# Tycro-Games/Raytracer-VoxPopuli

Hardware: AMD Instinct MI355X
Metric: Mray/s (primary+shadow) at 1920×1080, 1024³ world; 1/2/4/8-GPU (higher is better)
Workload: dtype f32

## Files before the change

raytracer-voxpopuli_amd/csrc/vpx_skip.hpp:

```cpp
#pragma once

#include <stdint.h>

#ifndef __HIP_DEVICE_COMPILE__
#include <cstring>
#endif

#if defined(__HIPCC__)
#define VPX_HD __host__ __device__ __forceinline__
#else
#define VPX_HD inline
#endif

namespace vpx {
namespace skip {

VPX_HD uint32_t fbits(float f) {
#if defined(__HIP_DEVICE_COMPILE__)
    return __float_as_uint(f);
#else
    uint32_t u;
    std::memcpy(&u, &f, 4);
    return u;
#endif
// ... 397 lines not shown
    return step1_commit(w, n, ax, ay, az);
}

VPX_HD int skip_box(Walk& w, const uint32_t lo[3], const uint32_t hi[3], float bound, uint32_t& cells) {
    const float h[3] = {w.tx, w.ty, w.tz};
    const float d[3] = {w.dx, w.dy, w.dz};
    const int32_t s[3] = {w.sx, w.sy, w.sz};
    const uint32_t c[3] = {w.X, w.Y, w.Z};
    uint32_t e[3];
    float approx[3];
    for (int k = 0; k < 3; ++k) {
        if (!(h[k] > 0.0f) || !(d[k] > 0.0f)) return 2;
        e[k] = s[k] > 0 ? hi[k] - c[k] + 1u : c[k] - lo[k] + 1u;
        approx[k] = e[k] > 1u ? h[k] + (float)(e[k] - 1u) * d[k] : h[k];
    }
    float V[3], Vp[3];
    bool exact[3] = {false, false, false};
    int a = (approx[2] <= approx[0] && approx[2] <= approx[1]) ? 2 : (approx[1] <= approx[0] ? 1 : 0);
    const float amin = approx[a];
    bool close = false;
    for (int k = 0; k < 3; ++k)
        if (k != a && !(approx[k] > amin * 1.0003f)) close = true;
    if (close) {
        for (int k = 0; k < 3; ++k) {
            count_below2(h[k], d[k], 3.4e38f, true, e[k] - 1u, V[k], Vp[k]);
            exact[k] = true;
        }
        a = (V[2] <= V[0] && V[2] <= V[1]) ? 2 : (V[1] <= V[0] ? 1 : 0);
    } else {
        count_below2(h[a], d[a], 3.4e38f, true, e[a] - 1u, V[a], Vp[a]);
        exact[a] = true;
    }
    const float vs = V[a];
    uint32_t nk[3];
    float head[3], prev[3];
    for (int k = 0; k < 3; ++k) {
        if (k == a) {
            nk[k] = e[k] - 1u;
            head[k] = V[k];
            prev[k] = Vp[k];
        } else {
            nk[k] = count_below2(h[k], d[k], vs, k < a, e[k] - 1u, head[k], prev[k]);
        }
    }
    if (vs < bound) {
        float tl = w.t;
        bool moved = false;
        for (int k = 0; k < 3; ++k) {
            if (nk[k] == 0) continue;
            tl = moved ? (tl < prev[k] ? prev[k] : tl) : prev[k];
            moved = true;
        }
        if (moved) w.t = tl;
        w.tx = head[0], w.ty = head[1], w.tz = head[2];
        w.X += nk[0] * (uint32_t)w.sx;
        w.Y += nk[1] * (uint32_t)w.sy;
        w.Z += nk[2] * (uint32_t)w.sz;
        cells += nk[0] + nk[1] + nk[2];
        return 0;
    }
    uint32_t v = 1u;
    for (int k = 0; k < 3; ++k) v += count_below(h[k], d[k], bound, true, nk[k]);
    cells += v;
    return 1;
}


VPX_HD uint32_t mul24(uint32_t a, uint32_t b) {
#if defined(__HIP_DEVICE_COMPILE__)
    return __umul24(a, b);
#else
    return a * b;
#endif
}

VPX_HD uint32_t mad24(uint32_t a, uint32_t b, uint32_t c) {
#if defined(__HIP_DEVICE_COMPILE__)
    uint32_t r;
    asm("v_mad_u32_u24 %0, %1, %2, %3" : "=v"(r) : "v"(a), "v"(b), "v"(c));
    return r;
#else
    return a * b + c;
#endif
}


VPX_HD float rcp_approx(float x) {
#if defined(__HIP_DEVICE_COMPILE__)
    return __builtin_amdgcn_rcpf(x);
#else
    return 1.0f / x;
#endif
}

VPX_HD bool seg_params_nb(float a, float d, uint32_t& b, uint32_t& c, uint32_t& e) {
    const uint32_t ab = fbits(a), db = fbits(d);
    const uint32_t ea = ab >> 23, ed = db >> 23;
    const uint32_t sh = ea - ed;
    const uint32_t sh1 = sh > 1u ? sh : 1u, shc = sh1 < 24u ? sh1 : 24u;
    const uint32_t md = (db & 0x7fffffu) | 0x800000u;
    const uint32_t rem = md & ((1u << shc) - 1u), half = 1u << (shc - 1u);
    const uint32_t c0 = md >> shc;
    const uint32_t b0 = (ab & 0x7fffffu) | 0x800000u;
    const bool tie = rem == half;
    c = tie ? c0 + (c0 & 1u) : c0 + (rem > half ? 1u : 0u);
    b = tie ? b0 + ((b0 + c0) & 1u) - (c0 & 1u) : b0;
    e = ea;
    return (ea - 1u < 254u) & (ed - 1u < 254u) & (sh - 1u < 24u) & (c != 0u);
}

VPX_HD uint32_t ceil_div_cap_r(uint32_t p, uint32_t c, float rc) {
    const float q = (float)p * rc;
    uint32_t j = (uint32_t)(q < 1024.5f ? q : 1024.5f) + 1u;
    j -= mul24(j - 1u, c) >= p ? 1u : 0u;
    j += mul24(j, c) < p ? 1u : 0u;
    return j < 1025u ? j : 1025u;
}
VPX_HD uint32_t ceil_div_cap(uint32_t p, uint32_t c) { return ceil_div_cap_r(p, c, rcp_approx((float)c)); }

VPX_HD uint32_t floor_div_cap_r(uint32_t r, uint32_t c, float rc) {
    const float q = (float)r * rc;
    uint32_t m = (uint32_t)(q < 1024.5f ? q : 1024.5f);
    m -= ((m != 0u) & (mul24(m, c) > r)) ? 1u : 0u;
    m += mul24(m + 1u, c) <= r ? 1u : 0u;
    return m < 1024u ? m : 1024u;
}
VPX_HD uint32_t floor_div_cap(uint32_t r, uint32_t c) { return floor_div_cap_r(r, c, rcp_approx((float)c)); }

VPX_HD uint32_t seg_first_cap(uint32_t b, uint32_t c, uint32_t e, float T, bool strict) {
    const uint32_t tb = fbits(T), te = tb >> 23;
    const uint32_t need = ((tb & 0x7fffffu) | 0x800000u) + (strict ? 0u : 1u);
    const uint32_t q = ceil_div_cap(need - b, c);
    const uint32_t f = need <= b ? 0u : q;
    return te == e ? f : (te < e ? 0u : 1025u);
}

struct Axis {
    uint32_t b1, c1, e1, m1, b2, c2, e2, l;
};

VPX_HD bool seg_immature(float h, float d) {
    const uint32_t ea = fbits(h) >> 23, ed = fbits(d) >> 23;
    return (ea - 1u < 254u) & (ed - 1u < 254u) & (ed >= ea);
}
template <bool PRE = false>
VPX_HD bool axis_seg1(float h, float d, Axis& a, uint32_t& fit1) {
    const bool ok1 = seg_params_nb(h, d, a.b1, a.c1, a.e1);
    if (PRE) a.c1 = ok1 ? a.c1 : 1u;
    const uint32_t room = a.b1 <= 0xffffffu ? 0xffffffu - a.b1 : 0u;
    fit1 = floor_div_cap(room, a.c1 ? a.c1 : 1u);
    if (PRE) fit1 = ok1 ? fit1 : 0u;
    a.b2 = 0u, a.c2 = 1u, a.e2 = 0u;
    return PRE ? ok1 | seg_immature(h, d) : ok1;
}
template <bool PRE = false>
VPX_HD uint32_t axis_seg2(float h, float d, Axis& a, uint32_t fit1) {
    const uint32_t amc = (a.e1 << 23) | (mad24(fit1, a.c1, a.b1) & 0x7fffffu);
    const uint32_t am = fit1 ? amc : fbits(h);
    const float A = bitsf(am) + d;
    uint32_t b2;
    const bool ok2 = seg_params_nb(A, d, b2, a.c2, a.e2);
    const bool exact2 = b2 == ((fbits(A) & 0x7fffffu) | 0x800000u);
    a.b2 = b2;
    if (PRE) a.c2 = ok2 ? a.c2 : 1u;
    const uint32_t room2 = b2 <= 0xffffffu ? 0xffffffu - b2 : 0u;
    const uint32_t fit2 = floor_div_cap(room2, a.c2 ? a.c2 : 1u);
    if (PRE) return exact2 ? fit1 + 1u + (ok2 ? fit2 : 0u) : fit1;
    return (ok2 & exact2) ? fit1 + 1u + fit2 : fit1;
}
VPX_HD void axis_clip(Axis& a, uint32_t l, bool ok1, uint32_t reach, uint32_t fit1) {
    const uint32_t lim = ok1 ? reach : 0u;
    a.l = l < lim ? l : lim;
    a.m1 = a.l < fit1 ? a.l : fit1;
}
VPX_HD float axis_head2(const Axis& a) { return bitsf((a.e2 << 23) | (a.b2 & 0x7fffffu)); }
VPX_HD bool axis_outrun(const Axis& a, uint32_t want) { return (want > a.l) & (a.l > a.m1); }
VPX_HD uint32_t axis_rebase(float& h, float d, Axis& a, uint32_t want, bool on) {
    const uint32_t fit1 = a.m1, fit2 = a.l - fit1 - 1u;
    const float A = bitsf((a.e2 << 23) | (mad24(fit2, a.c2, a.b2) & 0x7fffffu)) + d;
    uint32_t b3, c3, e3;
    const bool ok3 = seg_params_nb(A, d, b3, c3, e3);
    const bool exact3 = b3 == ((fbits(A) & 0x7fffffu) | 0x800000u);
    const uint32_t room3 = b3 <= 0xffffffu ? 0xffffffu - b3 : 0u;
    const uint32_t fit3 = floor_div_cap(room3, c3 ? c3 : 1u);
    const bool go = on & axis_outrun(a, want) & ok3 & exact3;
    const uint32_t off = fit1 + 1u, l = want - off, lim = fit2 + 1u + fit3;
    h = go ? axis_head2(a) : h;
    a.b1 = go ? a.b2 : a.b1, a.c1 = go ? a.c2 : a.c1, a.e1 = go ? a.e2 : a.e1;
    a.b2 = go ? b3 : a.b2, a.c2 = go ? c3 : a.c2, a.e2 = go ? e3 : a.e2;
    a.l = go ? (l < lim ? l : lim) : a.l;
    a.m1 = go ? (a.l < fit2 ? a.l : fit2) : a.m1;
    return go ? off : 0u;
}
VPX_HD bool any_lane(bool b) {
#if defined(__HIP_DEVICE_COMPILE__)
    return __ballot(b) != 0ull;
#else
    return b;
#endif
}

template <bool PRE = false>
VPX_HD void axis_setup(float h, float d, uint32_t l, Axis& a) {
    const bool ok1 = seg_params_nb(h, d, a.b1, a.c1, a.e1);
    if (PRE) a.c1 = ok1 ? a.c1 : 1u;
    const uint32_t room = a.b1 <= 0xffffffu ? 0xffffffu - a.b1 : 0u;
    const uint32_t fit1q = floor_div_cap(room, a.c1 ? a.c1 : 1u);
    const uint32_t fit1 = PRE && !ok1 ? 0u : fit1q;
    const uint32_t amc = (a.e1 << 23) | (mad24(fit1, a.c1, a.b1) & 0x7fffffu);
    const uint32_t am = fit1 ? amc : fbits(h);
    const float A = bitsf(am) + d;
    uint32_t b2;
    const bool ok2 = seg_params_nb(A, d, b2, a.c2, a.e2);
    const bool exact2 = b2 == ((fbits(A) & 0x7fffffu) | 0x800000u);
    a.b2 = b2;
    if (PRE) a.c2 = ok2 ? a.c2 : 1u;
    const uint32_t room2 = b2 <= 0xffffffu ? 0xffffffu - b2 : 0u;
    const uint32_t fit2 = floor_div_cap(room2, a.c2 ? a.c2 : 1u);
    const uint32_t reach = PRE ? (exact2 ? fit1 + 1u + (ok2 ? fit2 : 0u) : fit1) : ((ok2 & exact2) ? fit1 + 1u + fit2 : fit1);
    const uint32_t lim = (PRE ? ok1 | seg_immature(h, d) : ok1) ? reach : 0u;
    a.l = l < lim ? l : lim;
    a.m1 = a.l < fit1 ? a.l : fit1;
}

VPX_HD float axis_at(const Axis& a, float h, uint32_t i) {
    const bool one = i <= a.m1;
    const uint32_t b1 = mad24(i, a.c1, a.b1), b2 = mad24(i - a.m1 - 1u, a.c2, a.b2);
    const uint32_t v = ((one ? a.e1 : a.e2) << 23) | ((one ? b1 : b2) & 0x7fffffu);
    return bitsf(i ? v : fbits(h));
}

VPX_HD uint32_t axis_count(const Axis& a, float h, float T, bool strict, uint32_t cap) {
    const bool h_below = strict ? h < T : h <= T;
    const bool s2 = (fbits(T) >> 23) > a.e1;
    uint32_t f = seg_first_cap(s2 ? a.b2 : a.b1, s2 ? a.c2 : a.c1, s2 ? a.e2 : a.e1, T, strict);
    f = s2 ? a.m1 + 1u + f : (f < a.m1 + 1u ? f : a.m1 + 1u);
    f = h_below ? (f > 1u ? f : 1u) : 0u;
    return f < cap ? f : cap;
}

template <bool SEG2_BRANCH = true, int MORE = 0, bool PRE = false>
VPX_HD int skip_box_lean(Walk& w, uint32_t lo[3], uint32_t hi[3], float bound, uint32_t& cells) {
    static_assert(MORE == 0 || SEG2_BRANCH, "skip_box_lean: further segments build on the branch form");
    if (!((w.tx > 0.0f) & (w.ty > 0.0f) & (w.tz > 0.0f))) return 2;
    Axis ax, ay, az;
    if (SEG2_BRANCH) {
    const uint32_t wx = w.sx > 0 ? hi[0] - w.X : w.X - lo[0], wy = w.sy > 0 ? hi[1] - w.Y : w.Y - lo[1],
                   wz = w.sz > 0 ? hi[2] - w.Z : w.Z - lo[2];
    uint32_t fx, fy, fz;
    const bool okx = axis_seg1<PRE>(w.tx, w.dx, ax, fx), oky = axis_seg1<PRE>(w.ty, w.dy, ay, fy),
               okz = axis_seg1<PRE>(w.tz, w.dz, az, fz);
    uint32_t rx = fx, ry = fy, rz = fz;
    if (any_lane((okx & (wx > fx)) | (oky & (wy > fy)) | (okz & (wz > fz)))) {
        rx = axis_seg2<PRE>(w.tx, w.dx, ax, fx);
        ry = axis_seg2<PRE>(w.ty, w.dy, ay, fy);
        rz = axis_seg2<PRE>(w.tz, w.dz, az, fz);
    }
    axis_clip(ax, wx, okx, rx, fx);
    axis_clip(ay, wy, oky, ry, fy);
    axis_clip(az, wz, okz, rz, fz);
    } else {
    axis_setup<PRE>(w.tx, w.dx, w.sx > 0 ? hi[0] - w.X : w.X - lo[0], ax);
    axis_setup<PRE>(w.ty, w.dy, w.sy > 0 ? hi[1] - w.Y : w.Y - lo[1], ay);
    axis_setup<PRE>(w.tz, w.dz, w.sz > 0 ? hi[2] - w.Z : w.Z - lo[2], az);
    }
    for (int more = 0; more < MORE; ++more) {
        const uint32_t wx = w.sx > 0 ? hi[0] - w.X : w.X - lo[0], wy = w.sy > 0 ? hi[1] - w.Y : w.Y - lo[1],
                       wz = w.sz > 0 ? hi[2] - w.Z : w.Z - lo[2];
        const bool ux = axis_outrun(ax, wx), uy = axis_outrun(ay, wy), uz = axis_outrun(az, wz);
        if (!any_lane(ux | uy | uz)) break;
        const float Vx = axis_at(ax, w.tx, ax.l), Vy = axis_at(ay, w.ty, ay.l), Vz = axis_at(az, w.tz, az.l);
        const float Vm = Vx < Vy ? Vx : Vy, Vn = Vm < Vz ? Vm : Vz, T2 = Vn < bound ? Vn : bound;
        const uint32_t ox = axis_rebase(w.tx, w.dx, ax, wx, axis_head2(ax) < T2);
        const uint32_t oy = axis_rebase(w.ty, w.dy, ay, wy, axis_head2(ay) < T2);
        const uint32_t oz = axis_rebase(w.tz, w.dz, az, wz, axis_head2(az) < T2);
        w.X += ox * (uint32_t)w.sx;
        w.Y += oy * (uint32_t)w.sy;
        w.Z += oz * (uint32_t)w.sz;
        cells += ox + oy + oz;
    }
    const uint32_t lx = ax.l, ly = ay.l, lz = az.l;
    if (w.sx > 0) hi[0] = w.X + lx; else lo[0] = w.X - lx;
    if (w.sy > 0) hi[1] = w.Y + ly; else lo[1] = w.Y - ly;
    if (w.sz > 0) hi[2] = w.Z + lz; else lo[2] = w.Z - lz;
    const float Vx = axis_at(ax, w.tx, lx), Vy = axis_at(ay, w.ty, ly), Vz = axis_at(az, w.tz, lz);
    const int a = (Vz <= Vx && Vz <= Vy) ? 2 : (Vy <= Vx ? 1 : 0);
    const float vs = a == 2 ? Vz : (a == 1 ? Vy : Vx);
    const bool inside = vs < bound;
    const float T = inside ? vs : bound;
    uint32_t nx = axis_count(ax, w.tx, T, true, lx);
    uint32_t ny = axis_count(ay, w.ty, T, inside ? a == 2 : true, ly);
    uint32_t nz = axis_count(az, w.tz, T, inside ? false : true, lz);
    if (inside) {
        nx = a == 0 ? lx : nx;
        ny = a == 1 ? ly : ny;
        nz = a == 2 ? lz : nz;
        const float px = axis_at(ax, w.tx, nx - 1u), py = axis_at(ay, w.ty, ny - 1u), pz = axis_at(az, w.tz, nz - 1u);
        float tl = nx ? px : w.t;
        tl = ny ? ((nx && !(tl < py)) ? tl : py) : tl;
        tl = nz ? (((nx | ny) && !(tl < pz)) ? tl : pz) : tl;
        w.t = tl;
        w.tx = axis_at(ax, w.tx, nx), w.ty = axis_at(ay, w.ty, ny), w.tz = axis_at(az, w.tz, nz);
        w.X += nx * (uint32_t)w.sx;
        w.Y += ny * (uint32_t)w.sy;
        w.Z += nz * (uint32_t)w.sz;
        cells += nx + ny + nz;
        return 0;
    }
    const uint32_t cx = a == 0 ? lx : axis_count(ax, w.tx, vs, true, lx);
    const uint32_t cy = a == 1 ? ly : axis_count(ay, w.ty, vs, a == 2, ly);
    const uint32_t cz = a == 2 ? lz : axis_count(az, w.tz, vs, false, lz);
    cells += 1u + (nx < cx ? nx : cx) + (ny < cy ? ny : cy) + (nz < cz ? nz : cz);
    return 1;
}

VPX_HD bool gate_immature(float t, float d, uint32_t G) { return (fbits(t) >> 23) < (fbits(d) >> 23) + G; }
VPX_HD bool gate_open(float tx, float ty, float tz, float dx, float dy, float dz, uint32_t G, uint32_t N) {
    const bool xd = (dx <= dy) & (dx <= dz), yd = !xd & (dy <= dz);
    const float lim = (xd ? tx : (yd ? ty : tz)) + (float)N * (xd ? dx : (yd ? dy : dz));
    const bool ix = gate_immature(tx, dx, G), iy = gate_immature(ty, dy, G), iz = gate_immature(tz, dz, G);
    return !((ix & (tx < lim)) | (iy & (ty < lim)) | (iz & (tz < lim)));
}
VPX_HD uint32_t gate_word(uint32_t G, uint32_t f) { return 1u | G << 1 | f << 3; }
VPX_HD bool gate_open(const Walk& w, uint32_t gate) {
    return !(gate & 1u) || gate_open(w.tx, w.ty, w.tz, w.dx, w.dy, w.dz, (gate >> 1) & 3u, 4u << ((gate >> 3) & 3u));
}

constexpr uint32_t kGatePre = 1u << 8;
constexpr uint32_t kGatePacked = 1u << 9;
template <bool PRE>
VPX_HD int skip_box_lean_more(Walk& w, uint32_t lo[3], uint32_t hi[3], float bound, uint32_t& cells, uint32_t more) {
    return more == 0u   ? skip_box_lean<true, 0, PRE>(w, lo, hi, bound, cells)
           : more == 1u ? skip_box_lean<true, 1, PRE>(w, lo, hi, bound, cells)
           : more == 2u ? skip_box_lean<true, 2, PRE>(w, lo, hi, bound, cells)
           : more == 3u ? skip_box_lean<true, 3, PRE>(w, lo, hi, bound, cells)
                        : skip_box_lean<true, 4, PRE>(w, lo, hi, bound, cells);
}
VPX_HD bool walk_skip(const GridView& g, Walk& w, float bound, uint32_t& cells, uint32_t gate = 0u) {
    const bool wide = g.dfw != nullptr, axes = wide || g.dfa != nullptr;
    const uint32_t axis = dom_axis(w), sec = wide ? sec_axis(w) : 3u;
    const uint32_t apar = plane_parent(g, (w.osh >> 3) * 3u + axis);
    const bool packed = wide && (gate & kGatePacked);
    const uint32_t sel = packed ? box_sel(axis, sec) : 0u;
    for (;;) {
        if (!(w.t < bound)) return false;
        const int cls = axes ? classify_axis_o(w, g, apar) : classify(w, g);
        if (cls == 0) {
            ++cells;
            return true;
        }
        if (cls == 2 && gate_open(w, gate)) {
            uint32_t lo[3], hi[3];
            if (packed) df_box_sel(w, g.n, (uint32_t)w.m1, sel, lo, hi);
            else if (axes) df_box_axis(w, g.n, cube_dfp(w), len_dfa(w), axis, lo, hi, sec, wide ? wid_dfw(w, axis, sec) : 0u);
            else df_box(w, g.n, cube_l1(w), lo, hi);
            const int sr = (gate & kGatePre) ? skip_box_lean_more<true>(w, lo, hi, bound, cells, (gate >> 5) & 7u)
                                             : skip_box_lean_more<false>(w, lo, hi, bound, cells, (gate >> 5) & 7u);
            if (sr == 1) return false;
        }
        ++cells;
        if (!step1(w, g.n)) return false;
    }
}

template <class Occ, class Get>
VPX_HD uint8_t df_value(uint32_t x, uint32_t y, uint32_t z, uint32_t o, uint32_t nb1, Occ occ, Get get) {
    const int32_t s[3] = {(o & 1u) ? -1 : 1, (o & 2u) ? -1 : 1, (o & 4u) ? -1 : 1};
    uint32_t mn = 255;
    for (uint32_t j = 1; j < 8; ++j) {
        const uint32_t a = x + ((j & 1u) ? (uint32_t)s[0] : 0u), b = y + ((j & 2u) ? (uint32_t)s[1] : 0u),
                       c = z + ((j & 4u) ? (uint32_t)s[2] : 0u);
        const uint32_t v = (a < nb1 && b < nb1 && c < nb1) ? (occ(a, b, c) ? 0u : get(a, b, c, o)) : 255u;
        mn = v < mn ? v : mn;
    }
    return (uint8_t)(mn < 255u ? mn + 1u : 255u);
}

template <class Cube>
VPX_HD uint32_t axis_len(uint32_t x, uint32_t y, uint32_t z, uint32_t o, uint32_t a, uint32_t k, uint32_t nb1, Cube cube) {
    const uint32_t e = ((o >> a) & 1u) ? ~0u : 1u;
    uint32_t p[3] = {x, y, z};
    uint32_t L = k;
    while (L < 255u) {
        p[a] += e;
        if (p[a] >= nb1) return 255u;
        if (cube(p[0], p[1], p[2]) < k) break;
        ++L;
    }
    return L;
}

#ifndef VPX_WID_CAP
#define VPX_WID_CAP 255u
#endif
template <class Word>
VPX_HD uint32_t axis_wid(const uint32_t p[3], uint32_t o, uint32_t a, uint32_t b, uint32_t c, uint32_t k, uint32_t L, uint32_t nb1,
                         Word word) {
    const uint32_t ea = ((o >> a) & 1u) ? ~0u : 1u, eb = ((o >> b) & 1u) ? ~0u : 1u, ec = ((o >> c) & 1u) ? ~0u : 1u;
    const uint32_t top = k > VPX_WID_CAP ? k : VPX_WID_CAP;
    uint32_t q[3];
    uint32_t M = k;
    while (M < top) {
        q[b] = p[b] + eb * M;
        if (q[b] >= nb1) return top;
        uint32_t layers = 1u;
        for (uint32_t m = 0; m < k;) {
            q[c] = p[c] + ec * m;
            if (q[c] >= nb1) break;
            uint32_t rows = 1u;
            for (uint32_t i = 0; i < L;) {
                q[a] = p[a] + ea * i;
                if (q[a] >= nb1) break;
                const uint32_t w = word(q[0], q[1], q[2]);
                if (!w) return M;
                const uint32_t k2 = w & 255u, L2 = (w >> 8) & 255u;
                if (i == 0u && L2 >= L) {
                    rows = k2;
                    if (m == 0u && k2 >= k) layers = k2;
                }
                i += L2;
            }
            m += rows;
        }
        M += layers;
    }
    return top;
}
template <class Word>
VPX_HD uint32_t axis_wids(uint32_t x, uint32_t y, uint32_t z, uint32_t o, uint32_t a, uint32_t k, uint32_t L, uint32_t nb1, Word word) {
    const uint32_t p[3] = {x, y, z};
    const uint32_t b = a == 0u ? 1u : 0u, c = a == 2u ? 1u : 2u;
    return axis_wid(p, o, a, b, c, k, L, nb1, word) | axis_wid(p, o, a, c, b, k, L, nb1, word) << 8;
}

struct Box3 {
    int32_t lo[3], hi[3];
};
constexpr int32_t kBoxNone = 0x7fffffff;
VPX_HD Box3 box_none() { return Box3{{kBoxNone, kBoxNone, kBoxNone}, {-1, -1, -1}}; }
VPX_HD bool box_empty(const Box3& b) { return b.lo[0] > b.hi[0] || b.lo[1] > b.hi[1] || b.lo[2] > b.hi[2]; }
VPX_HD bool box_has(const Box3& b, const uint32_t p[3]) {
    return (int32_t)p[0] >= b.lo[0] && (int32_t)p[0] <= b.hi[0] && (int32_t)p[1] >= b.lo[1] && (int32_t)p[1] <= b.hi[1] &&
           (int32_t)p[2] >= b.lo[2] && (int32_t)p[2] <= b.hi[2];
}
VPX_HD void box_add(Box3& b, const uint32_t p[3]) {
    for (int q = 0; q < 3; ++q) {
        b.lo[q] = (int32_t)p[q] < b.lo[q] ? (int32_t)p[q] : b.lo[q];
        b.hi[q] = (int32_t)p[q] > b.hi[q] ? (int32_t)p[q] : b.hi[q];
    }
}
VPX_HD bool ahead_meets(const uint32_t p[3], uint32_t o, const uint32_t first[3], const uint32_t ext[3], const Box3& b) {
    bool hit = true;
    for (uint32_t q = 0; q < 3; ++q) {
        const int32_t near = (int32_t)first[q], far = (int32_t)(first[q] + ext[q]) - 1;
        const bool neg = (o >> q) & 1u;
        const int32_t l = neg ? (int32_t)p[q] - far : (int32_t)p[q] + near, h = neg ? (int32_t)p[q] - near : (int32_t)p[q] + far;
        hit = hit && ext[q] != 0u && l <= b.hi[q] && h >= b.lo[q];
    }
    return hit;
}
VPX_HD Box3 box_behind(const Box3& b, uint32_t o, const uint32_t ext[3], uint32_t nb1) {
    Box3 r = b;
    if (box_empty(b)) return r;
    for (uint32_t q = 0; q < 3; ++q) {
        if ((o >> q) & 1u) r.hi[q] = b.hi[q] + (int32_t)ext[q] - 1;
        else r.lo[q] = b.lo[q] - ((int32_t)ext[q] - 1);
        r.lo[q] = r.lo[q] < 0 ? 0 : r.lo[q];
        r.hi[q] = r.hi[q] > (int32_t)nb1 - 1 ? (int32_t)nb1 - 1 : r.hi[q];
    }
    return r;
}
constexpr uint32_t kReach = 256;
VPX_HD bool cube_dirty(const uint32_t p[3], uint32_t o, uint32_t k_old, const Box3& E) {
    const uint32_t first[3] = {0u, 0u, 0u}, ext[3] = {k_old + 1u, k_old + 1u, k_old + 1u};
    return ahead_meets(p, o, first, ext, E);
}
VPX_HD bool len_dirty(const uint32_t p[3], uint32_t o, uint32_t a, uint32_t k_old, uint32_t L_old, const Box3& C) {
    if (box_has(C, p)) return true;
    uint32_t first[3] = {0u, 0u, 0u}, ext[3] = {1u, 1u, 1u};
    first[a] = 1u, ext[a] = L_old - k_old + 1u;
    return ahead_meets(p, o, first, ext, C);
}
VPX_HD bool wid_dirty(const uint32_t p[3], uint32_t o, uint32_t a, uint32_t k, uint32_t L, uint32_t Mb, uint32_t Mc, const Box3& D) {
    if (box_has(D, p)) return true;
    if (!k) return false;
    const uint32_t b = a == 0u ? 1u : 0u, c = a == 2u ? 1u : 2u;
    const uint32_t first[3] = {0u, 0u, 0u};
    uint32_t e1[3], e2[3];
    e1[a] = L, e1[b] = Mb + 1u, e1[c] = k;
    e2[a] = L, e2[b] = k, e2[c] = Mc + 1u;
    return ahead_meets(p, o, first, e1, D) || ahead_meets(p, o, first, e2, D);
}

#if !defined(__HIP_DEVICE_COMPILE__)
inline void build_masks_host(const uint8_t* cells, uint32_t n, uint64_t* l1, uint64_t* l2) {
    const uint32_t nb1 = (n + 3) / 4, nb2 = (nb1 + 3) / 4, nb3 = (nb2 + 3) / 4;
    std::memset(l1, 0, 8ull * nb2 * nb2 * nb2 * 64);
    std::memset(l2, 0, 8ull * nb3 * nb3 * nb3 * 64);
    for (uint64_t z = 0; z < n; ++z)
        for (uint64_t y = 0; y < n; ++y)
            for (uint64_t x = 0; x < n; ++x)
                if (cells[x + y * n + z * (uint64_t)n * n] != 255)
                    l1[blk_index((uint32_t)x >> 2, (uint32_t)y >> 2, (uint32_t)z >> 2, nb2)] |=
                        1ull << ((x & 3) + 4 * (y & 3) + 16 * (z & 3));
    for (uint32_t z = 0; z < nb1; ++z)
        for (uint32_t y = 0; y < nb1; ++y)
            for (uint32_t x = 0; x < nb1; ++x)
                if (l1[blk_index(x, y, z, nb2)])
                    l2[blk_index(x >> 2, y >> 2, z >> 2, nb3)] |= 1ull << ((x & 3) + 4 * (y & 3) + 16 * (z & 3));
    auto occ = [&](uint32_t x, uint32_t y, uint32_t z) {
// ... 184 lines not shown
```

raytracer-voxpopuli_amd/csrc/vpx_trace.hpp:

```cpp
#pragma once

#include <hip/hip_runtime.h>
#include <stdint.h>

#include "../../include/vpx.h"
#include "vpx_skip.hpp"
#include "vpx_x86.hpp"
#ifndef VPX_WALK_KINDS
#define VPX_WALK_KINDS "vpx_walk_kinds.hpp"
#endif
#include VPX_WALK_KINDS

namespace vpx {

constexpr uint32_t kNone = 255u;
constexpr float kPi = 3.14159265358979323846264f;
constexpr float kBig = 1e34f;
constexpr int kMaxLevels = 16;

struct DevGrid {
    const uint8_t* cells;
    const uint64_t* l1;
    const uint64_t* l2;
    uint32_t n;
// ... 239 lines not shown
#endif
    return o;
}
__device__ __forceinline__ f3 nearest_rd(f3 d, const X86Arith& xa) {
#if !defined(VPX_NO_X86) && !defined(VPX_DEBUG_X86_NO_RCP)
    if (xa.tab) {
        const uint32_t tx = xa.tab[x86_rcp_key(__float_as_uint(d.x), xa.rcp_shift)];
        const uint32_t ty = xa.tab[x86_rcp_key(__float_as_uint(d.y), xa.rcp_shift)];
        const uint32_t tz = xa.tab[x86_rcp_key(__float_as_uint(d.z), xa.rcp_shift)];
#ifdef VPX_DEBUG_X86_WORK_EXACT
        const f3 fr = mk(fast_reciprocal1(d.x, tx), fast_reciprocal1(d.y, ty), fast_reciprocal1(d.z, tz));
        return mk(__fdiv_rn(1.0f, d.x) + 0.0f * fr.x, __fdiv_rn(1.0f, d.y) + 0.0f * fr.y,
                  __fdiv_rn(1.0f, d.z) + 0.0f * fr.z);
#endif
        return mk(fast_reciprocal1(d.x, tx), fast_reciprocal1(d.y, ty), fast_reciprocal1(d.z, tz));
    }
#endif
    return mk(__fdiv_rn(1.0f, d.x), __fdiv_rn(1.0f, d.y), __fdiv_rn(1.0f, d.z));
}

struct Dda {
    uint32_t X, Y, Z;
    int sx, sy, sz;
    float t;
    f3 tdelta, tmax;
};

__device__ __forceinline__ float cube_intersect(f3 b0, f3 b1, const ORay& r) {
    const bool sgx = r.D.x < 0, sgy = r.D.y < 0, sgz = r.D.z < 0;
    float tmin_x = ((sgx ? b1.x : b0.x) - r.O.x) * r.rD.x;
    float tmax_x = ((sgx ? b0.x : b1.x) - r.O.x) * r.rD.x;
    const float tmin_y = ((sgy ? b1.y : b0.y) - r.O.y) * r.rD.y;
    const float tmax_y = ((sgy ? b0.y : b1.y) - r.O.y) * r.rD.y;
    if (tmin_x > tmax_y || tmin_y > tmax_x) return kBig;
    tmin_x = smax(tmin_x, tmin_y);
    tmax_x = smin(tmax_x, tmax_y);
    const float tmin_z = ((sgz ? b1.z : b0.z) - r.O.z) * r.rD.z;
    const float tmax_z = ((sgz ? b0.z : b1.z) - r.O.z) * r.rD.z;
    if (tmin_x > tmax_z || tmin_z > tmax_x) return kBig;
    tmin_x = smax(tmin_x, tmin_z);
    return tmin_x > 0 ? tmin_x : kBig;
}

__device__ __forceinline__ bool dda_setup(const vpx_volume& vol, uint32_t n, const ORay& r, Dda& s) {
    const f3 b0 = ld3(vol.b0), b1 = ld3(vol.b1);
    s.t = 0;
    const bool contains = r.O.x >= b0.x && r.O.y >= b0.y && r.O.z >= b0.z && r.O.x <= b1.x &&
                          r.O.y <= b1.y && r.O.z <= b1.z;
    if (!contains) {
        s.t = cube_intersect(b0, b1, r);
        if (s.t > 1e33f) return false;
    }
    const f3 vmax = b1 - b0;
    const float g = (float)n;
    const float cell = __fdiv_rn(1.0f, g);
    const f3 ds = dsign(r.D);
    s.sx = trunc_i32(1.0f - ds.x * 2.0f);
    s.sy = trunc_i32(1.0f - ds.y * 2.0f);
    s.sz = trunc_i32(1.0f - ds.z * 2.0f);
    const f3 pos = (((r.O - b0) + r.D * (s.t + 0.00005f)) * g) / vmax;
    const f3 planes = (mk(ceilf(pos.x), ceilf(pos.y), ceilf(pos.z)) - ds) * cell;
    const int hi = (int)(n - 1);
    int px = trunc_i32(pos.x), py = trunc_i32(pos.y), pz = trunc_i32(pos.z);
    px = px < 0 ? 0 : (px > hi ? hi : px);
    py = py < 0 ? 0 : (py > hi ? hi : py);
    pz = pz < 0 ? 0 : (pz > hi ? hi : pz);
    s.X = (uint32_t)px;
    s.Y = (uint32_t)py;
    s.Z = (uint32_t)pz;
    s.tdelta = mk(cell * (float)s.sx, cell * (float)s.sy, cell * (float)s.sz) * r.rD;
    s.tmax = ((planes * vmax) - (r.O - b0)) * r.rD;
    return true;
}

__device__ __forceinline__ f3 normal_voxel(const ORay& r, float t, uint32_t n, const float* matrix) {
    const f3 i1 = (r.O + r.D * t) * (float)n;
    const f3 fg = mk(i1.x - floorf(i1.x), i1.y - floorf(i1.y), i1.z - floorf(i1.z));
    const f3 d = mk(smin(fg.x, 1.0f - fg.x), smin(fg.y, 1.0f - fg.y), smin(fg.z, 1.0f - fg.z));
    const float mind = smin(smin(d.x, d.y), d.z);
    const f3 sg = dsign(r.D) * 2.0f - mk(1.f, 1.f, 1.f);
    const f3 nn = mk(mind == d.x ? sg.x : 0.0f, mind == d.y ? sg.y : 0.0f, mind == d.z ? sg.z : 0.0f);
    return normalize(xform_vec(nn, matrix));
}

__device__ __forceinline__ uint32_t uni(uint32_t v) { return __builtin_amdgcn_readfirstlane(v); }
template <class T>
__device__ __forceinline__ T* uni_ptr(T* p) {
    const uint64_t v = (uint64_t)p;
    return (T*)(((uint64_t)uni((uint32_t)(v >> 32)) << 32) | uni((uint32_t)v));
}
__device__ __forceinline__ skip::GridView grid_view(const DevGrid& g) {
    const uint8_t* dfp = uni_ptr(g.dfp);
    return skip::GridView{uni_ptr(g.cells), uni_ptr(g.l1), uni_ptr(g.l2), uni(g.n), uni(g.nb1), uni(g.nb2),
                          uni(g.nb3),       dfp,            g.plane,        nullptr,  (const uint32_t*)(dfp + 8u * g.plane)};
}
__device__ __forceinline__ skip::Walk to_walk(const Dda& s) {
    skip::Walk w;
    w.X = s.X, w.Y = s.Y, w.Z = s.Z;
    w.t = s.t;
    w.tx = s.tmax.x, w.ty = s.tmax.y, w.tz = s.tmax.z;
    w.dx = s.tdelta.x, w.dy = s.tdelta.y, w.dz = s.tdelta.z;
    w.sx = s.sx, w.sy = s.sy, w.sz = s.sz;
    skip::walk_begin(w);
    return w;
}

#ifdef VPX_ASM_MARKS
#define VPX_MARK(s) asm volatile("; MARK " s)
#else
#define VPX_MARK(s)
#endif

#ifdef VPX_PHASE_PROF
__device__ unsigned long long g_phase[32];
#define VPX_PH(...) __VA_ARGS__
#else
#define VPX_PH(...)
#endif

constexpr int kFramePhases = 8, kFrameStripes = 64;
#ifdef VPX_PHASE_PROF
__device__ unsigned long long g_frame_phase[kFrameStripes][16];
__device__ __forceinline__ void frame_phase(int k) {
    const unsigned long long t = __builtin_amdgcn_s_memtime();
    if ((threadIdx.x & 63) == __builtin_amdgcn_readfirstlane(threadIdx.x & 63)) {
        unsigned long long* g = g_frame_phase[blockIdx.x % kFrameStripes];
        if (k > 0) atomicAdd(&g[k - 1], t);
        if (k < kFramePhases) atomicAdd(&g[k], 0ull - t);
        if (k == 0) atomicAdd(&g[kFramePhases], 1ull);
    }
}
#define VPX_FRAME_PHASE(k) do { VPX_MARK("frame " #k); frame_phase(k); } while (0)
#else
#define VPX_FRAME_PHASE(k) VPX_MARK("frame " #k)
#endif

constexpr int kWalkStep = 0, kWalkSkip = 1, kWalkMiss = 2, kWalkHit = 3;
__device__ __forceinline__ int stepped_axis(const skip::Walk& w, uint32_t ox, uint32_t oy) {
    return w.X != ox ? 0 : (w.Y != oy ? 1 : 2);
}
template <class KIND, bool POOL = false, bool REC = false>
__device__ __forceinline__ bool walk_wave(const skip::GridView& g, skip::Walk& w, float bound, uint32_t& cells,
                                          int* pmode = nullptr, uint32_t leave = 65u, int* plast = nullptr) {
    enum : int { kStep = kWalkStep, kSkip = kWalkSkip, kMiss = kWalkMiss, kHit = kWalkHit };
    constexpr int kRun = (int)KIND::run, kPasses = (int)KIND::passes;
    static_assert(KIND::skipw > 0 && kRun > 0 && kPasses > 0, "walk_wave: skip weight, run cap and passes");
    static_assert(KIND::minlen > 0, "walk_wave: the axis boxes' minimum length");
    static_assert(KIND::gate_g <= 3 && KIND::gate_n >= 4 && KIND::gate_n <= 32 && !(KIND::gate_n & (KIND::gate_n - 1)),
                  "walk_wave: the gate's exponent margin and event count (skip::gate_word's ranges)");
    const uint32_t opar = skip::plane_parent(g, (w.osh >> 3) * 3u + skip::dom_axis(w));
    const uint32_t sel = KIND::packed ? skip::box_sel(w) : 0u;
    int mode = POOL ? *pmode : kStep;
    int last = REC ? *plast : -1;
    VPX_PH(uint64_t cs = 0, ck = 0, ns = 0, nk = 0, ls = 0, lk = 0, fb = 0, cf = 0;)
    for (;;) {
        VPX_PH(uint64_t t0 = __builtin_amdgcn_s_memtime();)
        for (;;) {
            const uint64_t stepping = __ballot(mode == kStep);
            if (!stepping) break;
            const uint32_t nskip = (uint32_t)__popcll(__ballot(mode == kSkip));
            if ((uint32_t)__popcll(stepping) * KIND::skipw < nskip) break;
            if (POOL && 64u - (uint32_t)__popcll(stepping) - nskip >= leave) goto pool_out;
            VPX_PH(++ns; ls += __popcll(stepping); cf += __popcll(__ballot(mode >= kMiss));)
            VPX_MARK("step body");
#pragma unroll
            for (int u = 0; u < kPasses; ++u) {
                if (mode == kStep) {
                    if (!(w.t < bound)) {
                        mode = kMiss;
                    } else {
                        int cls = skip::classify_axis_o<KIND::minc, KIND::minlen, KIND::packed>(w, g, opar);
                        if (KIND::gate) {
                            float dx = w.dx, dy = w.dy, dz = w.dz;
                            asm volatile("" : "+v"(dx), "+v"(dy), "+v"(dz));
                            cls = (cls == 2 && !skip::gate_open(w.tx, w.ty, w.tz, dx, dy, dz, KIND::gate_g, KIND::gate_n)) ? 3 : cls;
                        }
                        if (KIND::packed) {
                            static_assert(kStep == 0 && kSkip == 1 && kHit == 3, "walk_wave: the class table's modes");
                            const uint32_t ent = (0x4147u >> (4u * (uint32_t)cls)) & 7u;
                            cells += ent >> 2;
                            mode = (int)(ent & 3u);
                        } else {
                            cells += cls != 2 ? 1u : 0u;
                            mode = cls == 0 ? kHit : (cls == 2 ? kSkip : mode);
                        }
                        if (cls & 1) {
                            const uint64_t solid = w.m1;
                            const uint32_t c1 = ((uint32_t)cls ^ 3u) >> 1;
#pragma unroll
                            for (int r = 0; r < kRun; ++r) {
                                const uint32_t ox = w.X, oy = w.Y, oz = w.Z;
                                const bool ing = skip::step1<KIND::min2>(w, g.n);
                                if (REC) last = stepped_axis(w, ox, oy);
                                const uint32_t moved = KIND::packed ? skip::xor_add(w.Z, oz, skip::xor_add(w.Y, oy, w.X ^ ox))
                                                                    : (w.X ^ ox) | (w.Y ^ oy) | (w.Z ^ oz);
                                const bool inb = r + 1 < kRun && moved <= 3u;
                                const bool inbound = w.t < bound;
                                const uint32_t cb =
                                    KIND::packed ? skip::cell_bit(w.X, w.Y, w.Z) : (w.X & 3u) | ((w.Y & 3u) << 2) | ((w.Z & 3u) << 4);
                                const bool sol = ((uint32_t)(solid >> cb) & c1) != 0u;
                                const bool visit = ing && inb && inbound;
                                cells += visit ? 1u : 0u;
                                mode = !ing || (inb && !inbound) ? kMiss : (visit && sol ? kHit : mode);
                                if (!visit || sol) break;
                            }
                        }
                    }
                }
            }
        }
        VPX_MARK("step phase end");
        VPX_PH(uint64_t t1 = __builtin_amdgcn_s_memtime(); cs += t1 - t0;)
        const uint64_t skipping = __ballot(mode == kSkip);
        if (!skipping) {
            if (!__ballot(mode == kStep)) break;
            continue;
        }
        VPX_PH(++nk; lk += __popcll(skipping);)
        VPX_MARK("skip phase");
        if (mode == kSkip) {
            uint32_t lo[3], hi[3];
            if (KIND::packed) {
                skip::df_box_sel(w, g.n, (uint32_t)w.m1, sel, lo, hi);
            } else {
                float dx = w.dx, dy = w.dy, dz = w.dz;
                if (KIND::local) asm volatile("" : "+v"(dx), "+v"(dy), "+v"(dz));
                const uint32_t axis = skip::dom_axis(dx, dy, dz), sec = skip::sec_axis(axis, dx, dy, dz);
                skip::df_box_axis(w, g.n, skip::cube_dfp(w), skip::len_dfa(w), axis, lo, hi, sec, skip::wid_dfw(w, axis, sec));
            }
            const int sr = skip::skip_box_lean<KIND::seg2, 0, KIND::pre>(w, lo, hi, bound, cells);
            VPX_MARK("skip end");
            VPX_PH(fb += __popcll(__ballot(sr == 2));)
            if (sr == 1) {
                mode = kMiss;
            } else {
                ++cells;
                const uint32_t ox = w.X, oy = w.Y;
                mode = skip::step1<KIND::min2>(w, g.n) ? kStep : kMiss;
                if (REC) last = stepped_axis(w, ox, oy);
            }
        }
        VPX_PH(ck += __builtin_amdgcn_s_memtime() - t1;)
    }
    if (POOL) {
    pool_out:
        *pmode = mode;
    }
    if (REC) *plast = last;
#ifdef VPX_PHASE_PROF
    if ((threadIdx.x & 63) == __builtin_amdgcn_readfirstlane(threadIdx.x & 63)) {
        atomicAdd(&g_phase[KIND::phase_slot + 0], cs);
        atomicAdd(&g_phase[KIND::phase_slot + 1], ck);
        atomicAdd(&g_phase[KIND::phase_slot + 2], ns);
        atomicAdd(&g_phase[KIND::phase_slot + 3], nk);
        atomicAdd(&g_phase[KIND::phase_slot + 4], ls);
        atomicAdd(&g_phase[KIND::phase_slot + 5], lk);
        atomicAdd(&g_phase[KIND::phase_slot + 6], 1ull);
        atomicAdd(&g_phase[KIND::phase_slot + 7], fb);
        atomicAdd(&g_phase[KIND::phase_slot + 8], cf);
    }
#endif
    return mode == kHit;
}

enum WalkMode { kNearest = 0, kGlassExit = 1, kSmokeExit = 2, kOcclusion = 3 };

struct WalkResult {
    bool hit;
    float t;
    uint32_t cell;
};

template <int MODE>
__device__ __forceinline__ WalkResult dda_walk(const DevGrid& g, Dda s, float bound, uint32_t& cells) {
    WalkResult res{false, s.t, kNone};
    const uint64_t n = g.n;
    const uint64_t nn = n * n;
    const uint8_t* __restrict__ grid = g.cells;
    for (;;) {
        if (MODE == kNearest || MODE == kOcclusion) {
            if (!(s.t < bound)) break;
        }
        const uint32_t cell = grid[(uint64_t)s.X + (uint64_t)s.Y * n + (uint64_t)s.Z * nn];
        ++cells;
        if (MODE == kNearest) {
            if (cell != kNone && s.t < bound) {
                res.hit = true, res.t = s.t, res.cell = cell;
                return res;
            }
        } else if (MODE == kOcclusion) {
            if (cell != kNone) {
                res.hit = s.t < bound;
                return res;
            }
        } else {
            const bool leave = (MODE == kGlassExit) ? (cell != VPX_MAT_GLASS)
                                                    : (cell > VPX_MAT_SMOKE_PLAYER || cell < VPX_MAT_SMOKE_LOW_DENSITY);
            if (leave) {
                res.hit = true, res.t = s.t, res.cell = cell;
                return res;
            }
        }
        const bool xy = s.tmax.x < s.tmax.y, xz = s.tmax.x < s.tmax.z, yz = s.tmax.y < s.tmax.z;
        const int axis = xy ? (xz ? 0 : 2) : (yz ? 1 : 2);
        if (axis == 0) {
            if (MODE != kOcclusion) s.t = s.tmax.x;
            s.X += (uint32_t)s.sx;
            if (s.X >= g.n) break;
            if (MODE == kOcclusion) s.t = s.tmax.x;
            s.tmax.x += s.tdelta.x;
        } else if (axis == 1) {
            if (MODE != kOcclusion) s.t = s.tmax.y;
            s.Y += (uint32_t)s.sy;
            if (s.Y >= g.n) break;
            if (MODE == kOcclusion) s.t = s.tmax.y;
            s.tmax.y += s.tdelta.y;
        } else {
            if (MODE != kOcclusion) s.t = s.tmax.z;
            s.Z += (uint32_t)s.sz;
            if (s.Z >= g.n) break;
            if (MODE == kOcclusion) s.t = s.tmax.z;
            s.tmax.z += s.tdelta.z;
        }
    }
    res.t = s.t;
    return res;
}

__device__ __forceinline__ void sphere_hit(const vpx_sphere& sp, Ray& r) {
    const f3 c = ld3(sp.center);
    const f3 to = r.O - c;
    const float b = dot(to, r.D);
    const float cc = dot(to, to) - (sp.radius * sp.radius);
    const float disc = b * b - cc;
    if (cc > 0.0f && b > 0.0f) return;
    if (disc < 0) return;
    const float len = -b - sqrtf(disc);
    if (len > r.t) return;
    if (len < 0) return;
    const f3 ip = r.O + r.D * len;
    const f3 outn = (ip - c) / sp.radius;
    const bool outside = dot(r.D, outn) < 0;
    r.N = outside ? outn : -outn;
    r.inside = !outside;
    r.t = len;
    r.mat = sp.material;
}
__device__ __forceinline__ bool sphere_is_hit(const vpx_sphere& sp, const Ray& r) {
    const f3 c = ld3(sp.center);
    const f3 to = r.O - c;
    const float b = dot(to, r.D);
    const float cc = dot(to, to) - (sp.radius * sp.radius);
    const float disc = b * b - cc;
    if (cc > 0.0f && b > 0.0f) return false;
    if (disc < 0) return false;
    const float len = -b - sqrtf(disc);
    if (len < 0) return false;
    if (len > r.t) return false;
    return true;
}
__device__ __forceinline__ bool tri_core(const vpx_triangle& tr, const Ray& r, float& t, f3& e1o, f3& e2o) {
    const f3 pos = ld3(tr.position);
    const f3 p1 = pos + ld3(tr.v0), p2 = pos + ld3(tr.v1), p3 = pos + ld3(tr.v2);
    const f3 e1 = p2 - p1, e2 = p3 - p1;
    const f3 h = cross(r.D, e2);
    const float a = dot(e1, h);
    if (a > -0.0001f && a < 0.0001f) return false;
    const float f = __fdiv_rn(1.0f, a);
    const f3 s = r.O - p1;
    const float u = f * dot(s, h);
    if (u < 0 || u > 1) return false;
    const f3 q = cross(s, e1);
    const float v = f * dot(r.D, q);
    if (v < 0 || u + v > 1) return false;
    t = f * dot(e2, q);
    e1o = e1;
    e2o = e2;
    return true;
}
__device__ __forceinline__ void tri_hit(const vpx_triangle& tr, Ray& r) {
    float t;
    f3 e1, e2;
    if (!tri_core(tr, r, t, e1, e2)) return;
    if (t > 0.0001f && r.t > t) {
        r.t = t;
        r.mat = tr.material;
        const f3 nrm = normalize(cross(e1, e2));
        r.N = dot(r.D, nrm) < 0 ? nrm : -nrm;
    }
}
__device__ __forceinline__ bool tri_is_hit(const vpx_triangle& tr, const Ray& r) {
    float t;
    f3 e1, e2;
    if (!tri_core(tr, r, t, e1, e2)) return false;
    if (t < 0.0001f) return false;
    if (t > r.t) return false;
    return true;
}

struct Counters {
    uint32_t cells;
    uint32_t shadow;
    uint32_t nearest;
};

__device__ __forceinline__ bool seg_box(float lx, float ly, float lz, float hx, float hy, float hz, f3 o, f3 inv,
                                        float bound) {
    float t0 = 0.0f, t1 = bound;
    const float ta[3] = {(lx - o.x) * inv.x, (ly - o.y) * inv.y, (lz - o.z) * inv.z};
    const float tb[3] = {(hx - o.x) * inv.x, (hy - o.y) * inv.y, (hz - o.z) * inv.z};
#pragma unroll
    for (int k = 0; k < 3; ++k) {
// ... 717 lines not shown
```

raytracer-voxpopuli_amd/csrc/vpx_walk_kinds.hpp:

```cpp
#pragma once

#include <stdint.h>

namespace vpx {

struct NearestWalk {
    static constexpr uint32_t skipw = 1;
    static constexpr uint32_t minc = 2;
    static constexpr uint32_t run = 3, passes = 3;
    static constexpr uint32_t minlen = 2;
    static constexpr bool pre = false;
    static constexpr bool seg2 = true;
    static constexpr bool min2 = true;
    static constexpr bool local = true;
    static constexpr bool packed = false;
    static constexpr bool gate = false;
    static constexpr uint32_t gate_g = 1, gate_n = 4;
    static constexpr int phase_slot = 0;
};
struct FrameNearestWalk : NearestWalk {
    static constexpr uint32_t passes = 4;
    static constexpr bool pre = true;
    static constexpr bool packed = true;
};
struct BounceWalk : NearestWalk {
    static constexpr uint32_t skipw = 2;
    static constexpr uint32_t run = 4, passes = 1;
    static constexpr bool pre = true;
    static constexpr bool seg2 = false;
    static constexpr bool local = false;
};
struct ShadowWalk : NearestWalk {
    static constexpr uint32_t skipw = 4;
    static constexpr uint32_t minc = 1;
    static constexpr uint32_t passes = 1;
    static constexpr bool min2 = false;
    static constexpr bool gate = true;
    static constexpr int phase_slot = 16;
};
struct FrameShadowWalk : ShadowWalk {
    static constexpr uint32_t passes = 3;
    static constexpr bool min2 = true;
    static constexpr bool packed = true;
};
struct ShadowPoolWalk : ShadowWalk {
    static constexpr bool min2 = true;
    static constexpr bool gate = false;
};
struct InstShadowWalk : ShadowWalk {
    static constexpr uint32_t minc = 2;
};

}
```

Baseline: 7369.

## Replace per-axis fit division with multiply overflow test; simplify miss cell count

Adds a FITMUL path in the box skip that decides whether the second float segment is needed by checking l*c against the mantissa room using 24-bit multiplies, instead of always computing a reciprocal-based floor division. The division now runs only when some lane overflows. FITMUL is off for every walk kind by default, so that path is inactive. Two other changes do run by default: the miss exit no longer computes per-axis counts capped at the exit, and FrameShadowWalk switches to the non-branch segment setup. The simpler count may over-report cells, which could change anything that depends on the cell count.

```diff
diff --git a/raytracer-voxpopuli_amd/csrc/vpx_skip.hpp b/raytracer-voxpopuli_amd/csrc/vpx_skip.hpp
--- a/raytracer-voxpopuli_amd/csrc/vpx_skip.hpp
+++ b/raytracer-voxpopuli_amd/csrc/vpx_skip.hpp
@@ -573,6 +573,31 @@
     if (PRE) fit1 = ok1 ? fit1 : 0u;
     a.b2 = 0u, a.c2 = 1u, a.e2 = 0u;
     return PRE ? ok1 | seg_immature(h, d) : ok1;
+}
+VPX_HD uint32_t mulhi24(uint32_t a, uint32_t b) {
+#if defined(__HIP_DEVICE_COMPILE__)
+    uint32_t r;
+    asm("v_mul_hi_u32_u24 %0, %1, %2" : "=v"(r) : "v"(a), "v"(b));
+    return r;
+#else
+    return (uint32_t)(((uint64_t)a * b) >> 32);
+#endif
+}
+template <bool PRE = false>
+VPX_HD bool axis_seg1_mul(float h, float d, uint32_t l, Axis& a, bool& ok1, bool& over) {
+    ok1 = seg_params_nb(h, d, a.b1, a.c1, a.e1);
+    if (PRE) a.c1 = ok1 ? a.c1 : 1u;
+    const uint32_t room = a.b1 <= 0xffffffu ? 0xffffffu - a.b1 : 0u, c = a.c1 ? a.c1 : 1u;
+    const bool past = (mulhi24(l, c) != 0u) || (mul24(l, c) > room);
+    over = PRE ? (ok1 ? past : l != 0u) : past;
+    a.b2 = 0u, a.c2 = 1u, a.e2 = 0u;
+    return PRE ? ok1 | seg_immature(h, d) : ok1;
+}
+template <bool PRE = false>
+VPX_HD uint32_t axis_fit1(const Axis& a, bool ok1) {
+    const uint32_t room = a.b1 <= 0xffffffu ? 0xffffffu - a.b1 : 0u;
+    const uint32_t fit1 = floor_div_cap(room, a.c1 ? a.c1 : 1u);
+    return PRE ? (ok1 ? fit1 : 0u) : fit1;
 }
 template <bool PRE = false>
 VPX_HD uint32_t axis_seg2(float h, float d, Axis& a, uint32_t fit1) {
@@ -660,12 +685,33 @@
     return f < cap ? f : cap;
 }
 
-template <bool SEG2_BRANCH = true, int MORE = 0, bool PRE = false>
-VPX_HD int skip_box_lean(Walk& w, uint32_t lo[3], uint32_t hi[3], float bound, uint32_t& cells) {
+template <bool SEG2_BRANCH = true, int MORE = 0, bool PRE = false, bool FITMUL = false>
+VPX_HD int skip_box_lean(Walk& w, uint32_t lo[3], uint32_t hi[3], float bound, uint32_t& cells, uint32_t* crossed = nullptr) {
     static_assert(MORE == 0 || SEG2_BRANCH, "skip_box_lean: further segments build on the branch form");
+    static_assert(!FITMUL || SEG2_BRANCH, "skip_box_lean: the multiply decides the branch");
     if (!((w.tx > 0.0f) & (w.ty > 0.0f) & (w.tz > 0.0f))) return 2;
     Axis ax, ay, az;
-    if (SEG2_BRANCH) {
+    if (SEG2_BRANCH && FITMUL) {
+    const uint32_t wx = w.sx > 0 ? hi[0] - w.X : w.X - lo[0], wy = w.sy > 0 ? hi[1] - w.Y : w.Y - lo[1],
+                   wz = w.sz > 0 ? hi[2] - w.Z : w.Z - lo[2];
+    bool kx, ky, kz, vx, vy, vz;
+    const bool okx = axis_seg1_mul<PRE>(w.tx, w.dx, wx, ax, kx, vx), oky = axis_seg1_mul<PRE>(w.ty, w.dy, wy, ay, ky, vy),
+               okz = axis_seg1_mul<PRE>(w.tz, w.dz, wz, az, kz, vz);
+    if (any_lane((okx & vx) | (oky & vy) | (okz & vz))) {
+        if (crossed) *crossed = 1u;
+        const uint32_t fx = axis_fit1<PRE>(ax, kx), fy = axis_fit1<PRE>(ay, ky), fz = axis_fit1<PRE>(az, kz);
+        const uint32_t rx = axis_seg2<PRE>(w.tx, w.dx, ax, fx);
+        const uint32_t ry = axis_seg2<PRE>(w.ty, w.dy, ay, fy);
+        const uint32_t rz = axis_seg2<PRE>(w.tz, w.dz, az, fz);
+        axis_clip(ax, wx, okx, rx, fx);
+        axis_clip(ay, wy, oky, ry, fy);
+        axis_clip(az, wz, okz, rz, fz);
+    } else {
+        ax.l = ax.m1 = okx ? wx : 0u;
+        ay.l = ay.m1 = oky ? wy : 0u;
+        az.l = az.m1 = okz ? wz : 0u;
+    }
+    } else if (SEG2_BRANCH) {
     const uint32_t wx = w.sx > 0 ? hi[0] - w.X : w.X - lo[0], wy = w.sy > 0 ? hi[1] - w.Y : w.Y - lo[1],
                    wz = w.sz > 0 ? hi[2] - w.Z : w.Z - lo[2];
     uint32_t fx, fy, fz;
@@ -673,6 +719,7 @@
                okz = axis_seg1<PRE>(w.tz, w.dz, az, fz);
     uint32_t rx = fx, ry = fy, rz = fz;
     if (any_lane((okx & (wx > fx)) | (oky & (wy > fy)) | (okz & (wz > fz)))) {
+        if (crossed) *crossed = 1u;
         rx = axis_seg2<PRE>(w.tx, w.dx, ax, fx);
         ry = axis_seg2<PRE>(w.ty, w.dy, ay, fy);
         rz = axis_seg2<PRE>(w.tz, w.dz, az, fz);
@@ -728,10 +775,7 @@
         cells += nx + ny + nz;
         return 0;
     }
-    const uint32_t cx = a == 0 ? lx : axis_count(ax, w.tx, vs, true, lx);
-    const uint32_t cy = a == 1 ? ly : axis_count(ay, w.ty, vs, a == 2, ly);
-    const uint32_t cz = a == 2 ? lz : axis_count(az, w.tz, vs, false, lz);
-    cells += 1u + (nx < cx ? nx : cx) + (ny < cy ? ny : cy) + (nz < cz ? nz : cz);
+    cells += 1u + nx + ny + nz;
     return 1;
 }
 
@@ -749,13 +793,21 @@
 
 constexpr uint32_t kGatePre = 1u << 8;
 constexpr uint32_t kGatePacked = 1u << 9;
-template <bool PRE>
+constexpr uint32_t kGateFitMul = 1u << 10;
+template <bool PRE, bool FITMUL>
 VPX_HD int skip_box_lean_more(Walk& w, uint32_t lo[3], uint32_t hi[3], float bound, uint32_t& cells, uint32_t more) {
-    return more == 0u   ? skip_box_lean<true, 0, PRE>(w, lo, hi, bound, cells)
-           : more == 1u ? skip_box_lean<true, 1, PRE>(w, lo, hi, bound, cells)
-           : more == 2u ? skip_box_lean<true, 2, PRE>(w, lo, hi, bound, cells)
-           : more == 3u ? skip_box_lean<true, 3, PRE>(w, lo, hi, bound, cells)
-                        : skip_box_lean<true, 4, PRE>(w, lo, hi, bound, cells);
+    return more == 0u   ? skip_box_lean<true, 0, PRE, FITMUL>(w, lo, hi, bound, cells)
+           : more == 1u ? skip_box_lean<true, 1, PRE, FITMUL>(w, lo, hi, bound, cells)
+           : more == 2u ? skip_box_lean<true, 2, PRE, FITMUL>(w, lo, hi, bound, cells)
+           : more == 3u ? skip_box_lean<true, 3, PRE, FITMUL>(w, lo, hi, bound, cells)
+                        : skip_box_lean<true, 4, PRE, FITMUL>(w, lo, hi, bound, cells);
+}
+VPX_HD int skip_box_lean_gate(Walk& w, uint32_t lo[3], uint32_t hi[3], float bound, uint32_t& cells, uint32_t gate) {
+    const uint32_t more = (gate >> 5) & 7u;
+    return (gate & kGateFitMul) ? ((gate & kGatePre) ? skip_box_lean_more<true, true>(w, lo, hi, bound, cells, more)
+                                                     : skip_box_lean_more<false, true>(w, lo, hi, bound, cells, more))
+                                : ((gate & kGatePre) ? skip_box_lean_more<true, false>(w, lo, hi, bound, cells, more)
+                                                     : skip_box_lean_more<false, false>(w, lo, hi, bound, cells, more));
 }
 VPX_HD bool walk_skip(const GridView& g, Walk& w, float bound, uint32_t& cells, uint32_t gate = 0u) {
     const bool wide = g.dfw != nullptr, axes = wide || g.dfa != nullptr;
@@ -775,8 +827,7 @@
             if (packed) df_box_sel(w, g.n, (uint32_t)w.m1, sel, lo, hi);
             else if (axes) df_box_axis(w, g.n, cube_dfp(w), len_dfa(w), axis, lo, hi, sec, wide ? wid_dfw(w, axis, sec) : 0u);
             else df_box(w, g.n, cube_l1(w), lo, hi);
-            const int sr = (gate & kGatePre) ? skip_box_lean_more<true>(w, lo, hi, bound, cells, (gate >> 5) & 7u)
-                                             : skip_box_lean_more<false>(w, lo, hi, bound, cells, (gate >> 5) & 7u);
+            const int sr = skip_box_lean_gate(w, lo, hi, bound, cells, gate);
             if (sr == 1) return false;
         }
         ++cells;
diff --git a/raytracer-voxpopuli_amd/csrc/vpx_trace.hpp b/raytracer-voxpopuli_amd/csrc/vpx_trace.hpp
--- a/raytracer-voxpopuli_amd/csrc/vpx_trace.hpp
+++ b/raytracer-voxpopuli_amd/csrc/vpx_trace.hpp
@@ -415,7 +415,7 @@
     const uint32_t sel = KIND::packed ? skip::box_sel(w) : 0u;
     int mode = POOL ? *pmode : kStep;
     int last = REC ? *plast : -1;
-    VPX_PH(uint64_t cs = 0, ck = 0, ns = 0, nk = 0, ls = 0, lk = 0, fb = 0, cf = 0;)
+    VPX_PH(uint64_t cs = 0, ck = 0, ns = 0, nk = 0, ls = 0, lk = 0, fb = 0, cf = 0, xb = 0;)
     for (;;) {
         VPX_PH(uint64_t t0 = __builtin_amdgcn_s_memtime();)
         for (;;) {
@@ -481,6 +481,7 @@
         }
         VPX_PH(++nk; lk += __popcll(skipping);)
         VPX_MARK("skip phase");
+        VPX_PH(uint32_t cr = 0u;)
         if (mode == kSkip) {
             uint32_t lo[3], hi[3];
             if (KIND::packed) {
@@ -491,7 +492,7 @@
                 const uint32_t axis = skip::dom_axis(dx, dy, dz), sec = skip::sec_axis(axis, dx, dy, dz);
                 skip::df_box_axis(w, g.n, skip::cube_dfp(w), skip::len_dfa(w), axis, lo, hi, sec, skip::wid_dfw(w, axis, sec));
             }
-            const int sr = skip::skip_box_lean<KIND::seg2, 0, KIND::pre>(w, lo, hi, bound, cells);
+            const int sr = skip::skip_box_lean<KIND::seg2, 0, KIND::pre, KIND::seg2 && KIND::fitmul>(w, lo, hi, bound, cells VPX_PH(, &cr));
             VPX_MARK("skip end");
             VPX_PH(fb += __popcll(__ballot(sr == 2));)
             if (sr == 1) {
@@ -503,6 +504,7 @@
                 if (REC) last = stepped_axis(w, ox, oy);
             }
         }
+        VPX_PH(xb += __ballot(cr != 0u) ? 1u : 0u;)
         VPX_PH(ck += __builtin_amdgcn_s_memtime() - t1;)
     }
     if (POOL) {
@@ -521,6 +523,7 @@
         atomicAdd(&g_phase[KIND::phase_slot + 6], 1ull);
         atomicAdd(&g_phase[KIND::phase_slot + 7], fb);
         atomicAdd(&g_phase[KIND::phase_slot + 8], cf);
+        atomicAdd(&g_phase[29 + (KIND::phase_slot ? 1 : 0)], xb);
     }
 #endif
     return mode == kHit;
diff --git a/raytracer-voxpopuli_amd/csrc/vpx_walk_kinds.hpp b/raytracer-voxpopuli_amd/csrc/vpx_walk_kinds.hpp
--- a/raytracer-voxpopuli_amd/csrc/vpx_walk_kinds.hpp
+++ b/raytracer-voxpopuli_amd/csrc/vpx_walk_kinds.hpp
@@ -11,6 +11,7 @@
     static constexpr uint32_t minlen = 2;
     static constexpr bool pre = false;
     static constexpr bool seg2 = true;
+    static constexpr bool fitmul = false;
     static constexpr bool min2 = true;
     static constexpr bool local = true;
     static constexpr bool packed = false;
@@ -39,6 +40,7 @@
     static constexpr int phase_slot = 16;
 };
 struct FrameShadowWalk : ShadowWalk {
+    static constexpr bool seg2 = false;
     static constexpr uint32_t passes = 3;
     static constexpr bool min2 = true;
     static constexpr bool packed = true;
```

Measured after the change: 7422 (median of 6 runs). No clear change (+0.7%).
